# paroj/aruco

Measured on AMD Instinct MI355X. Metric: frames/sec at 1920×1080, higher is better.
Workload: dtype u8; 1 GPU; 1920x1080 synthetic stream, ~20 markers/frame, threshold+contour+decode+LINES, no pose (config 2); distinct_frames_per_gpu=1024, markers_rendered_per_frame=20, batches_in_flight=5, build=src=0ab799cac5660a2f flags=[], gpu_max_hw_queues=4, parallelism=frames sharded 1 stream/GPU

## Files before the change

aruco_amd/csrc/k_contours.hip:

```cpp
#include <algorithm>

#include "bits_tiles.h"
#include "internal.h"
#include "decode_device.h"

namespace ah {

__device__ __forceinline__ int first_dir(uint32_t m, int s_end) {
    int s = s_end;
    do {
        s = (s - 1) & 7;
        if ((m >> s) & 1) break;
    } while (s != s_end);
    return s == s_end ? -1 : s;
}

__device__ __forceinline__ bool run_rule_tiles(const uint64_t* __restrict__ tiles, int tnx, int x, int y, int hole) {
    int avail, avail_up;
    const uint64_t mid = tb_row64(tiles, tnx, x, y, &avail), up = tb_row64(tiles, tnx, x, y - 1, &avail_up);
    if (!hole) {
        int L = (~mid) ? __builtin_ctzll(~mid) : 64;
        L = min(L, avail);
        const int hi = min(L, avail - 1);
        const uint64_t m = hi >= 2 ? ((hi >= 63 ? ~0ull : ((1ull << (hi + 1)) - 1ull)) & ~3ull) : 0ull;
// ... 923 lines not shown
        }
    }
    __syncthreads();
    if (LDSP && !a.from_pool)
        for (int i = lane; i < count; i += WAVE) a.pool[cd.pool_off + i] = P[i];

    double eps = (double)count * 0.05;
    eps *= eps;
    int pos = 0, rs_start = 0;
    bool le_eps = false;
    const uint32_t* PW = (const uint32_t*)P;
    for (int it = 0; it < 3; it++) {
        pos = (pos + rs_start) % count;
        uint32_t bd, bk, maxd, kmax;
        scan_cyclic<false>(PW, count, pos + 1 == count ? 0 : pos + 1, count - 1, lane, PW[pos], 0u, bd, bk);
        wave_argmax_first(bd, bk, &maxd, &kmax);
        if (maxd > 0) rs_start = (int)kmax + 1;
        le_eps = (double)maxd <= eps;
    }
    int top = 0, outn = 0;
    bool reject = false;
    if (lane == 0) s_outn = 0;
    if (!le_eps) {
        int sl_start = pos % count;
        int sl_end = (rs_start + sl_start) % count;
        if (lane == 0) {
            s_stack[0][0] = sl_end, s_stack[0][1] = sl_start;
            s_stack[1][0] = sl_start, s_stack[1][1] = sl_end;
        }
        top = 2;
    } else {
        if (lane == 0) s_out[0] = P[pos];
        outn = 1;
    }
    __syncthreads();
    while (top > 0) {
        if (outn + top > 8) {
            reject = true;
            break;
        }
        --top;
        const int sl_start = s_stack[top][0], sl_end = s_stack[top][1];
        __syncthreads();
        const short2 ep = P[sl_end], sp = P[sl_start];
        int len = sl_end - sl_start;
        if (len <= 0) len += count;
        bool small;
        int split = 0;
        if (len > 1) {
            const int dx = ep.x - sp.x, dy = ep.y - sp.y;
            const uint32_t w = ((uint32_t)(-dy) & 0xFFFFu) | ((uint32_t)dx << 16);
            uint32_t bd, bq, maxd_u, qmax;
            scan_cyclic<true>(PW, count, sl_start + 1 == count ? 0 : sl_start + 1, len - 1, lane, PW[sl_start], w, bd, bq);
            wave_argmax_first(bd, bq, &maxd_u, &qmax);
            double maxd = (double)maxd_u;
            int q = qmax == 0xFFFFFFFFu ? 0 : (int)qmax;
            split = sl_start + 1 + q;
            if (split >= count) split -= count;
            small = maxd * maxd <= eps * ((double)dx * (double)dx + (double)dy * (double)dy);
        } else {
            small = true;
        }
        if (small) {
            if (lane == 0) s_out[outn] = sp;
            outn++;
        } else {
            if (lane == 0) {
                s_stack[top][0] = split, s_stack[top][1] = sl_end;
                s_stack[top + 1][0] = sl_start, s_stack[top + 1][1] = split;
            }
            top += 2;
        }
        __syncthreads();
    }
    if (reject || outn < 4) return;
    if (lane == 0) polygon_to_quad(a, cd, ci, s_out, outn, eps);
}

#ifndef DUAL_MAX_N
#define DUAL_MAX_N 512
#endif
constexpr int DUAL_MAX = DUAL_MAX_N;
__device__ __forceinline__ void border_pair_to_quads(const QuadArgs& a, const ContourDesc& cd, const uint32_t ci, const bool valid, short2* Pbase, int (*s_stack)[16][2],
                                                     short2 (*s_out)[12], uint32_t* rows) {
    const int lane = threadIdx.x, h = lane >> 5, hl = lane & 31;
    const bool upper = h != 0;
    short2* P = Pbase + h * DUAL_MAX;
    uint32_t* P32 = (uint32_t*)P;
    const int count = valid ? cd.n : 1;
    if (a.from_pool) {
        if (valid)
            for (int i = hl; i < count; i += 32) P[i] = a.pool[cd.pool_off + i];
    } else {
        const uint64_t* tiles = a.tiles + (size_t)cd.plane * a.tnx * a.tny;
        const int ncp = (count + CK - 1) / CK;
        const uint32_t* ckp = cd.ck_off == 0xFFFFFFFFu ? (const uint32_t*)(a.pool + cd.pool_off) - ncp : a.walk_scratch + cd.ck_off;
        const uint32_t* rb = rows + lane - 64;
        for (int k = hl; k < (DUAL_MAX + CK - 1) / CK; k += 32) {
            if (!(valid && k < ncp)) continue;
            const uint32_t c = ckp[k];
            const uint32_t pos = (c & 0x3FFFu) | (((c >> 14) & 0x3FFFu) << 16);
            const int n0 = k * CK, n1 = min(n0 + CK, count);
            int bx, by;
            if (k + 1 < ncp) {
                const uint32_t cn = ckp[k + 1];
                bx = (int)(cn & 0x3FFFu), by = (int)((cn >> 14) & 0x3FFFu);
            } else {
                bx = cd.x0, by = cd.y0;
            }
            const int ax = (int)(pos & 0xFFFFu), ay = (int)(pos >> 16), L = n1 - n0;
            const int ex = (L - abs(bx - ax)) >> 1, ey = (L - abs(by - ay)) >> 1;
            const int tx0 = min(max((min(ax, bx) - ex - 1) >> 3, 0), a.tnx - 4), ty0 = min(max((min(ay, by) - ey - 1) >> 3, 0), a.tny - 4);
            TileBlock blk;
            tb_load_at<64>(tiles, a.tnx, tx0, ty0, rows, lane, blk);
            const uint32_t base1 = tb_base1(blk);
            uint32_t lp = pos - base1, s1c = tb_s1c((int)(c >> 28));
#pragma unroll
            for (int j = 0; j < CK; j++) {
                if (n0 + j < n1) {
                    P32[n0 + j] = lp + base1;
                    tb_step<64>(rb, lp, s1c);
                }
            }
        }
    }
    __syncthreads();
    if (!a.from_pool && valid)
        for (int i = hl; i < count; i += 32) a.pool[cd.pool_off + i] = P[i];

    double eps = (double)count * 0.05;
    eps *= eps;
    int pos = 0, rs_start = 0;
    bool le_eps = false;
    const uint32_t* PW = (const uint32_t*)P;
    for (int it = 0; it < 3; it++) {
        pos = (pos + rs_start) % count;
        uint32_t bd, bk, maxd, kmax;
        scan_cyclic<false, 32>(PW, count, pos + 1 == count ? 0 : pos + 1, count - 1, hl, PW[pos], 0u, bd, bk);
        half_argmax_first(bd, bk, upper, &maxd, &kmax);
        if (maxd > 0) rs_start = (int)kmax + 1;
        le_eps = (double)maxd <= eps;
    }
    int top = 0, outn = 0;
    bool reject = !valid;
    if (!le_eps) {
        const int sl_start = pos % count;
        const int sl_end = (rs_start + sl_start) % count;
        if (hl == 0) {
            s_stack[h][0][0] = sl_end, s_stack[h][0][1] = sl_start;
            s_stack[h][1][0] = sl_start, s_stack[h][1][1] = sl_end;
        }
        top = 2;
    } else {
        if (hl == 0) s_out[h][0] = P[pos];
        outn = 1;
    }
    __syncthreads();
    for (;;) {
        bool act = !reject && top > 0;
        if (act && outn + top > 8) reject = true, act = false;
        if (!__any(act)) break;
        int sl_start = 0, sl_end = 0, len = 0;
        short2 ep = make_short2(0, 0), sp = make_short2(0, 0);
        uint32_t bd = 0, bq = 0xFFFFFFFFu;
        int dx = 0, dy = 0;
        if (act) {
            --top;
            sl_start = s_stack[h][top][0], sl_end = s_stack[h][top][1];
            ep = P[sl_end], sp = P[sl_start];
            len = sl_end - sl_start;
            if (len <= 0) len += count;
            if (len > 1) {
                dx = ep.x - sp.x, dy = ep.y - sp.y;
                const uint32_t w = ((uint32_t)(-dy) & 0xFFFFu) | ((uint32_t)dx << 16);
                scan_cyclic<true, 32>(PW, count, sl_start + 1 == count ? 0 : sl_start + 1, len - 1, hl, PW[sl_start], w, bd, bq);
            }
        }
        __syncthreads();
        uint32_t maxd_u, qmax;
        half_argmax_first(bd, bq, upper, &maxd_u, &qmax);
        if (act) {
            bool small = true;
            int split = 0;
            if (len > 1) {
                const double maxd = (double)maxd_u;
                const int q = qmax == 0xFFFFFFFFu ? 0 : (int)qmax;
                split = sl_start + 1 + q;
                if (split >= count) split -= count;
                small = maxd * maxd <= eps * ((double)dx * (double)dx + (double)dy * (double)dy);
            }
            if (small) {
                if (hl == 0) s_out[h][outn] = sp;
                outn++;
            } else {
                if (hl == 0) {
                    s_stack[h][top][0] = split, s_stack[h][top][1] = sl_end;
                    s_stack[h][top + 1][0] = sl_start, s_stack[h][top + 1][1] = split;
                }
                top += 2;
            }
        }
        __syncthreads();
    }
    if (hl == 0 && !reject && outn >= 4) polygon_to_quad(a, cd, ci, s_out[h], outn, eps);
}

__device__ __forceinline__ void quad_blocks(const QuadArgs& a, const int bid, short2* Plds, uint32_t* rows, int (*s_stack)[16][2], short2 (*s_out)[12], int& s_outn) {
    const int xcd = bid & 7, rest = bid >> 3;
    const int chunk = rest % a.qblocks, plane = (rest / a.qblocks) * 8 + xcd;
    if (plane >= a.nplanes) return;
    const uint32_t nall = min(a.trig_cnt[plane * TRIG_CNT_STRIDE + TC_CDESC], a.cap_cdesc);
    const uint32_t nsnap = min(a.trig_cnt[plane * TRIG_CNT_STRIDE + TC_SNAP], a.cap_cdesc);
    const uint32_t nlate = a.pass == 3 ? min(a.trig_cnt[plane * TRIG_CNT_STRIDE + TC_LATE], a.cap_cdesc - nall) : 0u;
    const uint32_t lo = a.pass == 2 ? nsnap : 0u, ncd = a.pass == 3 ? nlate : a.pass == 1 ? nsnap : nall;
    const bool upper = threadIdx.x >= 32;
    ContourDesc pend;
    uint32_t pend_ci = 0;
    bool has_pend = false;
    for (uint32_t cslot = lo + (uint32_t)chunk; cslot < ncd; cslot += (uint32_t)a.qblocks) {
        const uint32_t ci = (uint32_t)plane * a.cap_cdesc + (a.pass == 3 ? a.cap_cdesc - 1u - cslot : cslot);
        const ContourDesc cd = a.cdesc[ci];
        if (cd.n <= 0) continue;
        if (a.dual && cd.n <= DUAL_MAX) {
            if (!has_pend) {
                pend = cd, pend_ci = ci, has_pend = true;
                continue;
            }
            __syncthreads();
            border_pair_to_quads(a, upper ? cd : pend, upper ? ci : pend_ci, true, Plds, s_stack, s_out, rows);
            has_pend = false;
            continue;
        }
        __syncthreads();
        if (cd.n <= QP_LDS)
            border_to_quad<true>(a, cd, ci, Plds, s_stack[0], s_out[0], s_outn, rows);
        else
            border_to_quad<false>(a, cd, ci, a.pool + cd.pool_off, s_stack[0], s_out[0], s_outn, rows);
    }
    if (has_pend) {
        __syncthreads();
        border_to_quad<true>(a, pend, pend_ci, Plds, s_stack[0], s_out[0], s_outn, rows);
    }
}

__global__ __launch_bounds__(64) void contour_quad_kernel(QuadArgs a) {
    throughput_bound_priority();
    __shared__ __align__(16) short2 Plds[QP_LDS];
    __shared__ uint32_t rows[TB_ROWS * EMIT_LANES];
    __shared__ int s_stack[2][16][2];
    __shared__ short2 s_out[2][12];
    __shared__ int s_outn;
    static_assert(QP_LDS >= 2 * DUAL_MAX && EMIT_LANES == 64, "the two-borders-per-wave path uses the whole point buffer and a block per lane");
    quad_blocks(a, blockIdx.x, Plds, rows, s_stack, s_out, s_outn);
}

struct LateQuadArgs {
    WalkArgs w;
    QuadArgs q;
};
__global__ __launch_bounds__(64) void late_quad_kernel(LateQuadArgs a) {
    __shared__ __align__(16) short2 Plds[QP_LDS];
    __shared__ uint32_t rows[TB_ROWS * EMIT_LANES];
    __shared__ int s_stack[2][16][2];
    __shared__ short2 s_out[2][12];
    __shared__ int s_outn;
    static_assert(EMIT_LANES == 64, "the late walks use the quad role's blocks: one per lane");
    const int nwalk = 2 * a.w.gen_blocks;
    if ((int)blockIdx.x < nwalk) {
        latency_bound_priority();
        if ((int)blockIdx.x < a.w.gen_blocks)
            walk_generation<false, true>(a.w, blockIdx.x, rows);
        else
            walk_generation<true, true>(a.w, blockIdx.x - a.w.gen_blocks, rows);
        return;
    }
    throughput_bound_priority();
    quad_blocks(a.q, (int)blockIdx.x - nwalk, Plds, rows, s_stack, s_out, s_outn);
}

static int quad_blocks_per_plane(int nplanes) {
    constexpr int kBlocks = 12;
    return nplanes <= 2 ? 128 : nplanes <= 8 ? 48 : kBlocks;
}

static QuadArgs quad_args(const FrameGeom& g, int nframes, const DetectParams& p, const Buffers& b, int pass) {
    QuadArgs a;
    a.pass = pass;
    a.tiles = b.tiles, a.tnx = tiles_x(g.width), a.tny = tiles_y(g.height), a.from_pool = b.seg_mode, a.cdesc = b.cdesc, a.pool = b.pool, a.quads = b.quads, a.counters = b.counters;
    a.cap_cdesc = b.cap_cdesc, a.cap_quads = b.cap_quads, a.nthr = p.nthr, a.width = g.width, a.height = g.height;
    a.trig_cnt = b.trig_cnt, a.walk_scratch = b.walk_scratch;
    a.nplanes = nframes * p.nthr;
    a.dual = b.env.quad_dual && a.nplanes > 8;
    const int qb = quad_blocks_per_plane(a.nplanes);
    a.qblocks = pass == 2 ? std::max(1, qb / 2) : qb;
    return a;
}

void launch_contour_quads(hipStream_t s, const FrameGeom& g, int nframes, const DetectParams& p, const Buffers& b, int pass) {
    const QuadArgs a = quad_args(g, nframes, p, b, pass);
    const int planes8 = ((a.nplanes + 7) / 8) * 8;
    hipLaunchKernelGGL(contour_quad_kernel, dim3(planes8 * a.qblocks), dim3(64), 0, s, a);
}

void launch_late_quads(hipStream_t s, const FrameGeom& g, int nframes, const DetectParams& p, const Buffers& b) {
    LateQuadArgs a;
    a.w = walk_args(g, nframes * p.nthr, p, b);
    a.w.gen = GEN_FORK_AFTER + 1, a.w.gen_steps = p.max_contour;
    int before = a.w.leash;
    for (int gen = 1; gen <= GEN_FORK_AFTER; gen++) before += gen_steps_of(gen, p);
    a.w.gen_blocks = gen_blocks_of(a.w.nplanes, before);
    a.q = quad_args(g, nframes, p, b, 0);
    const int planes8 = ((a.q.nplanes + 7) / 8) * 8;
    hipLaunchKernelGGL(late_quad_kernel, dim3(2 * a.w.gen_blocks + planes8 * a.q.qblocks), dim3(64), 0, s, a);
    launch_contour_quads(s, g, nframes, p, b, 3);
}

struct FrameArgs {
    double* iM;
    int ws;
    const Quad* quads;
    Cand* cands;
    uint32_t* cand_list;
    uint32_t cap_flat;
    int32_t* ncands;
    uint32_t* counters;
    uint32_t* trig_cnt;
    int nthr;
    int cap_quads, cap_cands;
};

constexpr int MAXQ = 512;

__device__ __forceinline__ float quad_perimeter_i(const int16_t* x, const int16_t* y) {
    float sum = 0;
    for (int i = 0; i < 4; i++) {
        int j = (i + 1) & 3;
        double dx = (double)(x[i] - x[j]), dy = (double)(y[i] - y[j]);
        sum = (float)((double)sum + sqrt(dx * dx + dy * dy));
    }
    return sum;
}

template <int HG>
__global__ __launch_bounds__(64) void frame_candidates_kernel(FrameArgs a) {
    latency_bound_priority();
    constexpr int PHASE1_BYTES = MAXQ * (8 + 8 + 4 + 4 + 2 + 1 + 1);
    constexpr int BIG_DOUBLES = homography_lds_doubles<HG>() > (PHASE1_BYTES + 7) / 8 ? homography_lds_doubles<HG>() : (PHASE1_BYTES + 7) / 8;
    __shared__ double s_big[BIG_DOUBLES];
    int16_t(*sx)[4] = (int16_t(*)[4])s_big;
    int16_t(*sy)[4] = sx + MAXQ;
    int* s_cdesc = (int*)(sy + MAXQ);
    float* s_perim = (float*)(s_cdesc + MAXQ);
    int16_t* s_map = (int16_t*)(s_perim + MAXQ);
    uint8_t* s_swapped = (uint8_t*)(s_map + MAXQ);
    uint8_t* s_rem = s_swapped + MAXQ;
    __shared__ int s_n;
    __shared__ uint32_t s_base;
    const int frame = blockIdx.x, lane = threadIdx.x;
    const int nq = min((int)a.counters[CNT_FIXED + frame], min(a.cap_quads, MAXQ));
    const Quad* Q = a.quads + (size_t)frame * a.cap_quads;
    for (int i = lane; i < nq; i += WAVE) {
        const uint32_t key = Q[i].key;
        int rank = 0;
        for (int j = 0; j < nq; j++) rank += Q[j].key < key;
        Quad q = Q[i];
        int d1x = q.x[1] - q.x[0], d1y = q.y[1] - q.y[0], d2x = q.x[2] - q.x[0], d2y = q.y[2] - q.y[0];
        float o = ((float)d1x * (float)d2y) - ((float)d1y * (float)d2x);
        bool sw = o < 0.0f;
        if (sw) {
            int16_t tx = q.x[1], ty = q.y[1];
            q.x[1] = q.x[3], q.y[1] = q.y[3];
            q.x[3] = tx, q.y[3] = ty;
        }
        for (int k = 0; k < 4; k++) sx[rank][k] = q.x[k], sy[rank][k] = q.y[k];
        s_cdesc[rank] = q.cdesc;
        s_swapped[rank] = sw;
        s_rem[rank] = 0;
        s_perim[rank] = quad_perimeter_i(q.x, q.y);
    }
    __syncthreads();
    for (int i = 0; i < nq; i++) {
        for (int j = i + 1 + lane; j < nq; j += WAVE) {
            bool near = true;
            for (int c = 0; c < 4; c++) {
                int dx = sx[i][c] - sx[j][c], dy = sy[i][c] - sy[j][c];
                near = near && (dx * dx + dy * dy < 36);
            }
            if (near) {
                if (s_perim[i] > s_perim[j])
                    s_rem[j] = 1;
                else
                    s_rem[i] = 1;
            }
        }
    }
    __syncthreads();
    if (lane == 0) {
        int n = 0;
        Cand* C = a.cands + (size_t)frame * a.cap_cands;
        for (int i = 0; i < nq; i++) {
            if (s_rem[i]) continue;
            if (n >= a.cap_cands) {
                flag_overflow(a.counters, a.trig_cnt, frame * a.nthr, ST_CAND_OVERFLOW);
                break;
            }
            Cand c;
            for (int k = 0; k < 4; k++) {
                c.c[2 * k] = (float)sx[i][k], c.c[2 * k + 1] = (float)sy[i][k];
                c.qx[k] = sx[i][k], c.qy[k] = sy[i][k];
            }
            c.cdesc = s_cdesc[i], c.swapped = s_swapped[i], c.id = -1, c.nrot = 0;
            s_map[n] = (int16_t)i;
            C[n++] = c;
        }
        a.ncands[frame] = n;
        uint32_t base = 0;
        if (n > 0) {
            base = atomicAdd(&a.counters[CNT_NCAND], (uint32_t)n);
            for (int i = 0; i < n; i++) {
                if (base + i < a.cap_flat)
                    a.cand_list[base + i] = ((uint32_t)frame << 16) | (uint32_t)i;
                else
                    flag_overflow(a.counters, a.trig_cnt, frame * a.nthr, ST_CAND_OVERFLOW);
            }
        }
        s_n = n, s_base = base;
    }
    __syncthreads();
    const int n = s_n;
    const uint32_t base = s_base;
    constexpr int PER_LANE = MAXQ / WAVE;
    int16_t qx[PER_LANE][4], qy[PER_LANE][4];
#pragma unroll
    for (int r = 0; r < PER_LANE; r++) {
        const int k = r * WAVE + lane;
        if (k < n) {
            const int i = s_map[k];
            for (int c = 0; c < 4; c++) qx[r][c] = sx[i][c], qy[r][c] = sy[i][c];
        } else {
            for (int c = 0; c < 4; c++) qx[r][c] = 0, qy[r][c] = 0;
        }
    }
    __syncthreads();
    const LaneMatT<HG> A{s_big, lane}, b{s_big + 64 * HG, lane};
#pragma unroll
    for (int r = 0; r < PER_LANE; r++) {
        if (r * WAVE >= n) break;
        const int k = r * WAVE + lane;
        for (int g = 0; g < WAVE / HG; g++) {
            if (r * WAVE + g * HG >= n) break;
            if (lane / HG == g && k < n && base + (uint32_t)k < a.cap_flat)
                homography_lane(qx[r], qy[r], a.ws, A, b, a.iM + (size_t)(base + (uint32_t)k) * 9);
        }
    }
}

void launch_frame_candidates(hipStream_t s, const FrameGeom& g, int nframes, const DetectParams& p, const Buffers& b) {
    FrameArgs a;
    a.quads = b.quads, a.cands = b.cands, a.ncands = b.ncands, a.counters = b.counters, a.trig_cnt = b.trig_cnt, a.nthr = p.nthr;
    a.cand_list = b.cand_list, a.cap_flat = b.cap_flat;
    a.cap_quads = b.cap_quads, a.cap_cands = b.cap_cands;
    a.iM = b.iM, a.ws = p.warp_size;
    if (nframes <= 2)
        hipLaunchKernelGGL(frame_candidates_kernel<64>, dim3(nframes), dim3(64), 0, s, a);
    else
        hipLaunchKernelGGL(frame_candidates_kernel<HOMOGRAPHY_GROUP>, dim3(nframes), dim3(64), 0, s, a);
}

}
```

Baseline: 443,100 frames/s.

## Process late border contours with dedicated 256-thread block-cooperative quad kernel

Replaces the single-wave pass-3 contour quad launch for late (long) contours with a new kernel using 256-thread workgroups. Each block stages contour points in LDS, reconstructs chunked chain codes cooperatively, and runs the Douglas-Peucker-style simplification with block-wide argmax reductions. Block count per plane is set separately. The aim is to speed up the long-contour tail, at the cost of extra __syncthreads and larger LDS use that may cut occupancy.

```diff
diff --git a/aruco_amd/csrc/k_contours.hip b/aruco_amd/csrc/k_contours.hip
--- a/aruco_amd/csrc/k_contours.hip
+++ b/aruco_amd/csrc/k_contours.hip
@@ -1249,6 +1249,186 @@
     hipLaunchKernelGGL(contour_quad_kernel, dim3(planes8 * a.qblocks), dim3(64), 0, s, a);
 }
 
+constexpr int LB_THREADS = 256;
+constexpr int LB_WAVES = LB_THREADS / WAVE;
+#ifndef LB_LDS_N
+#define LB_LDS_N 7680
+#endif
+constexpr int LB_LDS = LB_LDS_N;
+
+#ifndef LB_SMALL_EMIT_N
+#define LB_SMALL_EMIT_N 64
+#endif
+constexpr int LB_SMALL = 3840, LB_SMALL_EMIT = LB_SMALL_EMIT_N;
+
+__device__ __forceinline__ void block_argmax_first(uint32_t val, uint32_t idx, uint32_t (*s_red)[2], uint32_t* max_val, uint32_t* first_idx) {
+    uint32_t wv, wi;
+    wave_argmax_first(val, idx, &wv, &wi);
+    if ((threadIdx.x & (WAVE - 1)) == 0) s_red[threadIdx.x / WAVE][0] = wv, s_red[threadIdx.x / WAVE][1] = wi;
+    __syncthreads();
+    uint32_t mv = 0;
+#pragma unroll
+    for (int w = 0; w < LB_WAVES; w++) mv = max(mv, s_red[w][0]);
+    uint32_t mi = 0xFFFFFFFFu;
+#pragma unroll
+    for (int w = 0; w < LB_WAVES; w++)
+        if (s_red[w][0] == mv) mi = min(mi, s_red[w][1]);
+    *max_val = mv, *first_idx = mi;
+}
+
+template <bool LDSP, int EMIT>
+__device__ __forceinline__ void late_border_to_quad(const QuadArgs& a, const ContourDesc& cd, const uint32_t ci, short2* P, uint32_t* rows, int (*s_stack)[2], short2* s_out,
+                                                    uint32_t (*s_red)[LB_WAVES][2]) {
+    const int lane = threadIdx.x;
+    const int count = cd.n;
+    if (a.from_pool) {
+        if (LDSP)
+            for (int i = lane; i < count; i += LB_THREADS) P[i] = a.pool[cd.pool_off + i];
+    } else {
+        const uint64_t* tiles = a.tiles + (size_t)cd.plane * a.tnx * a.tny;
+        const int ncp = (count + CK - 1) / CK;
+        const uint32_t* ckp = cd.ck_off == 0xFFFFFFFFu ? (const uint32_t*)(a.pool + cd.pool_off) - ncp : a.walk_scratch + cd.ck_off;
+        uint32_t* P32 = (uint32_t*)P;
+        const uint32_t* rb = rows + lane - EMIT;
+        for (int k0 = 0; k0 < ncp; k0 += EMIT) {
+            const int k = k0 + lane;
+            if (lane >= EMIT || k >= ncp) continue;
+            const uint32_t c = ckp[k];
+            const uint32_t pos = (c & 0x3FFFu) | (((c >> 14) & 0x3FFFu) << 16);
+            const int n0 = k * CK, n1 = min(n0 + CK, count);
+            int bx, by;
+            if (k + 1 < ncp) {
+                const uint32_t cn = ckp[k + 1];
+                bx = (int)(cn & 0x3FFFu), by = (int)((cn >> 14) & 0x3FFFu);
+            } else {
+                bx = cd.x0, by = cd.y0;
+            }
+            const int ax = (int)(pos & 0xFFFFu), ay = (int)(pos >> 16), L = n1 - n0;
+            const int ex = (L - abs(bx - ax)) >> 1, ey = (L - abs(by - ay)) >> 1;
+            const int tx0 = min(max((min(ax, bx) - ex - 1) >> 3, 0), a.tnx - 4), ty0 = min(max((min(ay, by) - ey - 1) >> 3, 0), a.tny - 4);
+            TileBlock blk;
+            tb_load_at<EMIT>(tiles, a.tnx, tx0, ty0, rows, lane, blk);
+            const uint32_t base1 = tb_base1(blk);
+            uint32_t lp = pos - base1, s1c = tb_s1c((int)(c >> 28));
+#pragma unroll
+            for (int j = 0; j < CK; j++) {
+                if (n0 + j < n1) {
+                    P32[n0 + j] = lp + base1;
+                    tb_step<EMIT>(rb, lp, s1c);
+                }
+            }
+        }
+    }
+    __syncthreads();
+    if (LDSP && !a.from_pool)
+        for (int i = lane; i < count; i += LB_THREADS) a.pool[cd.pool_off + i] = P[i];
+
+    double eps = (double)count * 0.05;
+    eps *= eps;
+    int pos = 0, rs_start = 0, par = 0;
+    bool le_eps = false;
+    const uint32_t* PW = (const uint32_t*)P;
+    for (int it = 0; it < 3; it++) {
+        pos = (pos + rs_start) % count;
+        uint32_t bd, bk, maxd, kmax;
+        scan_cyclic<false, LB_THREADS>(PW, count, pos + 1 == count ? 0 : pos + 1, count - 1, lane, PW[pos], 0u, bd, bk);
+        block_argmax_first(bd, bk, s_red[par], &maxd, &kmax);
+        par ^= 1;
+        if (maxd > 0) rs_start = (int)kmax + 1;
+        le_eps = (double)maxd <= eps;
+    }
+    int top = 0, outn = 0;
+    bool reject = false;
+    if (!le_eps) {
+        int sl_start = pos % count;
+        int sl_end = (rs_start + sl_start) % count;
+        if (lane == 0) {
+            s_stack[0][0] = sl_end, s_stack[0][1] = sl_start;
+            s_stack[1][0] = sl_start, s_stack[1][1] = sl_end;
+        }
+        top = 2;
+    } else {
+        if (lane == 0) s_out[0] = P[pos];
+        outn = 1;
+    }
+    __syncthreads();
+    while (top > 0) {
+        if (outn + top > 8) {
+            reject = true;
+            break;
+        }
+        --top;
+        const int sl_start = s_stack[top][0], sl_end = s_stack[top][1];
+        const short2 ep = P[sl_end], sp = P[sl_start];
+        int len = sl_end - sl_start;
+        if (len <= 0) len += count;
+        bool small;
+        int split = 0;
+        if (len > 1) {
+            const int dx = ep.x - sp.x, dy = ep.y - sp.y;
+            const uint32_t w = ((uint32_t)(-dy) & 0xFFFFu) | ((uint32_t)dx << 16);
+            uint32_t bd, bq, maxd_u, qmax;
+            scan_cyclic<true, LB_THREADS>(PW, count, sl_start + 1 == count ? 0 : sl_start + 1, len - 1, lane, PW[sl_start], w, bd, bq);
+            block_argmax_first(bd, bq, s_red[par], &maxd_u, &qmax);
+            par ^= 1;
+            double maxd = (double)maxd_u;
+            int q = qmax == 0xFFFFFFFFu ? 0 : (int)qmax;
+            split = sl_start + 1 + q;
+            if (split >= count) split -= count;
+            small = maxd * maxd <= eps * ((double)dx * (double)dx + (double)dy * (double)dy);
+        } else {
+            small = true;
+        }
+        if (small) {
+            if (lane == 0) s_out[outn] = sp;
+            outn++;
+        } else {
+            if (lane == 0) {
+                s_stack[top][0] = split, s_stack[top][1] = sl_end;
+                s_stack[top + 1][0] = sl_start, s_stack[top + 1][1] = split;
+            }
+            top += 2;
+        }
+        __syncthreads();
+    }
+    if (reject || outn < 4) return;
+    if (lane == 0) polygon_to_quad(a, cd, ci, s_out, outn, eps);
+}
+
+template <int PTS, int EMIT>
+__global__ __launch_bounds__(LB_THREADS) void late_border_quad_kernel(QuadArgs a) {
+    latency_bound_priority();
+    __shared__ __align__(16) short2 Plds[PTS];
+    __shared__ uint32_t rows[TB_ROWS * EMIT];
+    __shared__ int s_stack[16][2];
+    __shared__ short2 s_out[12];
+    __shared__ uint32_t s_red[2][LB_WAVES][2];
+    static_assert(EMIT % WAVE == 0 && EMIT <= LB_THREADS && sizeof(short2) * PTS + sizeof(uint32_t) * TB_ROWS * EMIT + 512 <= 65536, "a workgroup's static LDS stays within 64 KB");
+    const int bid = blockIdx.x, xcd = bid & 7, rest = bid >> 3;
+    const int chunk = rest % a.qblocks, plane = (rest / a.qblocks) * 8 + xcd;
+    if (plane >= a.nplanes) return;
+    const uint32_t nall = min(a.trig_cnt[plane * TRIG_CNT_STRIDE + TC_CDESC], a.cap_cdesc);
+    const uint32_t nlate = min(a.trig_cnt[plane * TRIG_CNT_STRIDE + TC_LATE], a.cap_cdesc - nall);
+    for (uint32_t cslot = (uint32_t)chunk; cslot < nlate; cslot += (uint32_t)a.qblocks) {
+        const uint32_t ci = (uint32_t)plane * a.cap_cdesc + a.cap_cdesc - 1u - cslot;
+        const ContourDesc cd = a.cdesc[ci];
+        if (cd.n <= 0) continue;
+        __syncthreads();
+        if (cd.n <= PTS)
+            late_border_to_quad<true, EMIT>(a, cd, ci, Plds, rows, s_stack, s_out, s_red);
+        else
+            late_border_to_quad<false, EMIT>(a, cd, ci, a.pool + cd.pool_off, rows, s_stack, s_out, s_red);
+    }
+}
+
+#ifndef LATE_BLOCKS_N
+#define LATE_BLOCKS_N 4
+#endif
+static int late_blocks_per_plane(int nplanes) {
+    constexpr int kBlocks = LATE_BLOCKS_N;
+    return nplanes <= 8 ? 16 : kBlocks;
+}
+
 void launch_late_quads(hipStream_t s, const FrameGeom& g, int nframes, const DetectParams& p, const Buffers& b) {
     LateQuadArgs a;
     a.w = walk_args(g, nframes * p.nthr, p, b);
@@ -1259,7 +1439,12 @@
     a.q = quad_args(g, nframes, p, b, 0);
     const int planes8 = ((a.q.nplanes + 7) / 8) * 8;
     hipLaunchKernelGGL(late_quad_kernel, dim3(2 * a.w.gen_blocks + planes8 * a.q.qblocks), dim3(64), 0, s, a);
-    launch_contour_quads(s, g, nframes, p, b, 3);
+    QuadArgs l = quad_args(g, nframes, p, b, 3);
+    l.qblocks = late_blocks_per_plane(l.nplanes);
+    if (p.max_contour <= LB_SMALL)
+        hipLaunchKernelGGL((late_border_quad_kernel<LB_SMALL, LB_SMALL_EMIT>), dim3(planes8 * l.qblocks), dim3(LB_THREADS), 0, s, l);
+    else
+        hipLaunchKernelGGL((late_border_quad_kernel<LB_LDS, LB_THREADS>), dim3(planes8 * l.qblocks), dim3(LB_THREADS), 0, s, l);
 }
 
 struct FrameArgs {
```

After: 437,100 frames/s. -1.4%, worse.
